# jbrea/BayesianOptimization.jl

Measured on AMD Instinct MI355X. Metric: acquisition-candidates/sec (N=3000,d=8), higher is better.
Workload: dtype f64

## Files before the change

### bayesianoptimization.jl_amd/csrc/kernels_score.hip

```cpp
#include "gemm_core.h"
#include "acq_log.h"

namespace bohip {

template <bool LOW>
__device__ __forceinline__ double cov_from_r_fast(int fam, double sigma2, double r) {
    if constexpr (LOW) {
        return matern_lo_k(fam, sigma2, r);
    } else {
        if (fam == FAM_M52) {
            const double R = sqrt(r), s = sqrt(5.0) * R;
            return sigma2 * (1.0 + s + 5.0 / 3.0 * r) * exp(-s);
        }
        return sigma2 * exp(-0.5 * r);
    }
}

struct KstarParts {
    const double* alpha;
    double* parts;
    int64_t ldp;
};
template <int DT, bool LOW>
__device__ __forceinline__ double kstar_value(const double (&xj)[DT], const double (&w)[DT], const double* xs, bool live, int fam,
                                              double sigma2) {
    double rr = 0.0;
#pragma unroll
    for (int k = 0; k < DT; ++k) {
        const double t = xj[k] - xs[k];
        rr += w[k] * (t * t);
    }
    return live ? cov_from_r_fast<LOW>(fam, sigma2, rr) : 0.0;
}
__device__ __forceinline__ void swap32(double a, double b, double& x, double& y) {
    const unsigned long long ua = (unsigned long long)__double_as_longlong(a), ub = (unsigned long long)__double_as_longlong(b);
    const auto lo = __builtin_amdgcn_permlane32_swap((unsigned)ua, (unsigned)ub, false, false);
    const auto hi = __builtin_amdgcn_permlane32_swap((unsigned)(ua >> 32), (unsigned)(ub >> 32), false, false);
    x = __longlong_as_double((long long)((unsigned long long)hi[0] << 32 | lo[0]));
    y = __longlong_as_double((long long)((unsigned long long)hi[1] << 32 | lo[1]));
}
template <int BIT>
__device__ __forceinline__ double halve_sum(double a, double b, int lane) {
    const bool up = lane & BIT;
    return (up ? b : a) + __shfl_xor(up ? a : b, BIT);
}
__device__ __forceinline__ void group_sum4(const double* p, int lane, double& sm, double& sa) {
    double x0, y0, x1, y1;
    swap32(p[0], p[2], x0, y0);
    swap32(p[1], p[3], x1, y1);
    sm = halve_sum<16>(x0 + y0, x1 + y1, lane);
    sa = halve_sum<16>(fabs(x0) + fabs(y0), fabs(x1) + fabs(y1), lane);
}
__device__ __forceinline__ double wave_finish(double s) {
    s += __shfl_xor(s, 2);
    s += __shfl_xor(s, 1);
    return s;
}

template <int DT, bool LOW, bool PARTS = false>
__global__ __launch_bounds__(256) void k_kstar(const double* __restrict__ X, int64_t N, int64_t Npad,
                                               const double* __restrict__ Xs, int64_t r_begin, int64_t r_end,
                                               KernelHyper hp, double* __restrict__ KsT, int64_t ldk, int rb, KstarParts kp) {
    __shared__ double xs_l[16 * DT];
    const int d = hp.d;
    const int64_t j = blockIdx.x * 256 + threadIdx.x;
    const int64_t r0 = r_begin + (int64_t)blockIdx.y * rb;
    const int64_t r1 = min(r0 + rb, r_end);
    for (int t = threadIdx.x; t < rb * DT; t += 256) {
        const int64_t r = r0 + t / DT;
        const int k = t % DT;
        xs_l[t] = (r < r1 && k < d) ? Xs[r * d + k] : 0.0;
    }
    double xj[DT], w[DT];
#pragma unroll
    for (int k = 0; k < DT; ++k) {
        xj[k] = (k < d && j < N) ? X[j * d + k] : 0.0;
        w[k] = k < d ? hp.il2[k] : 0.0;
    }
    __syncthreads();
    if (j >= Npad) return;
    const int nc = (int)(r1 - r0);
    if constexpr (PARTS) {
        const double aj = kp.alpha[j];
        const int lane = threadIdx.x & 63;
        double um[2], ua[2], tm0 = 0.0, ta0 = 0.0;
#pragma unroll
        for (int g = 0; g < 4; ++g) {
            double p[4];
#pragma unroll
            for (int i = 0; i < 4; ++i) {
                const int c = 4 * g + i;
                p[i] = 0.0;
                if (c < nc) {
                    const double v = kstar_value<DT, LOW>(xj, w, xs_l + c * DT, j < N, hp.fam, hp.sigma2);
                    KsT[(r0 + c - r_begin) * ldk + j] = v;
                    p[i] = aj * v;
                }
            }
            double tm, ta;
            group_sum4(p, lane, tm, ta);
            if (g & 1) {
                um[g >> 1] = halve_sum<8>(tm0, tm, lane);
                ua[g >> 1] = halve_sum<8>(ta0, ta, lane);
            } else {
                tm0 = tm;
                ta0 = ta;
            }
            __builtin_amdgcn_sched_barrier(0);
        }
        const double sm = wave_finish(halve_sum<4>(um[0], um[1], lane)), sa = wave_finish(halve_sum<4>(ua[0], ua[1], lane));
        const int c = 8 * ((lane >> 2) & 1) + 4 * ((lane >> 3) & 1) + 2 * (lane >> 5) + ((lane >> 4) & 1);
        if ((lane & 3) < 2 && c < nc) {
            const int64_t P = Npad >> 6;
            kp.parts[((int64_t)(lane & 1) * P + (j >> 6)) * kp.ldp + (r0 + c - r_begin)] = (lane & 1) ? sa : sm;
        }
    } else {
        for (int c = 0; c < nc; ++c) {
            const double v = kstar_value<DT, LOW>(xj, w, xs_l + c * DT, j < N, hp.fam, hp.sigma2);
            KsT[(r0 + c - r_begin) * ldk + j] = v;
        }
    }
}

template <int DT, bool LOW>
__global__ __launch_bounds__(256) void k_post_cov(const double* __restrict__ Xs, int64_t R, KernelHyper hp,
                                                  const double* __restrict__ VV, int64_t ldv,
                                                  double* __restrict__ cov, int64_t ldc) {
    const int d = hp.d;
    const int64_t s = blockIdx.x * 256 + threadIdx.x;
    if (s >= R) return;
    double xs[DT];
#pragma unroll
    for (int k = 0; k < DT; ++k) xs[k] = (k < d) ? Xs[s * d + k] : 0.0;
    const int64_t r0 = (int64_t)blockIdx.y * 16, r1 = min(R, r0 + 16);
    for (int64_t r = r0; r < r1; ++r) {
        double rr = 0.0;
#pragma unroll
        for (int k = 0; k < DT; ++k)
            if (k < d) {
                const double t = Xs[r * d + k] - xs[k];
                rr += hp.il2[k] * (t * t);
            }
        const double vv = (r >= s) ? VV[r * ldv + s] : VV[s * ldv + r];
        cov[r * ldc + s] = cov_from_r_fast<LOW>(hp.fam, hp.sigma2, rr) - vv;
    }
}

struct AcqParams {
    int acq;
    double p0, p1;
};
struct FuseParams {
    unsigned* tile_cnt;
    unsigned* total_cnt;
    Best* tile_best;
    int tiles_total;
    int T;
    int64_t R_total;
    double sigma2, beta;
    AcqParams ap;
    double *mu_out, *var_out, *score_out;
    Best* best_out;
    long long best_off;
    unsigned long long* clk;
    const unsigned* live;
};
__device__ void trigemm_fused_finish(const FuseParams& fz, int tile_g, int T, const double* q_part, int64_t ldq,
                                     const double* mu_raw);

#if BOHIP_TRACE
__device__ unsigned long long g_trace[6 * 8192];
#endif
constexpr int PIECE_WHOLE = 0, PIECE_UPPER_SOLO = 3;

__device__ __forceinline__ double sq_step(double s, double v) { return s + v * v; }
__device__ __forceinline__ double sq_tree(double s) {
    s += __shfl_xor(s, 8);
    s += __shfl_xor(s, 16);
    s += __shfl_xor(s, 32);
    return s;
}

__device__ __forceinline__ void trigemm_job(int rt, int mode, int ct, const double* __restrict__ W, int64_t ldw,
                                            const double* __restrict__ KsT, int64_t ldk, int NP, int64_t alpha_row,
                                            double* __restrict__ q_part, int64_t ldq, double* __restrict__ mu_raw, int64_t r_off,
                                            double* __restrict__ VT, int64_t ldv, const FuseParams& fz, double* smem, int tid) {
    constexpr int NJ = 4, CW = CTILE;
    double acc[8][NJ];
#pragma unroll
    for (int i = 0; i < 8; ++i)
#pragma unroll
        for (int j = 0; j < NJ; ++j) acc[i][j] = 0.0;
    const int64_t row_base = (int64_t)rt * TILE;
    const int active_rows = (int)min((int64_t)(mode == PIECE_WHOLE ? TILE : TILE / 2), alpha_row + 1 - row_base);
    const int tri_kc = rt * (TILE / KC);
    const int kc_end = mode == PIECE_WHOLE ? (rt + 1) * (TILE / KC) : tri_kc + 4;
    gemm_tile_loop_glds3_ks<NJ, BOHIP_ABL, true>(W + row_base * ldw, ldw, KsT + (int64_t)ct * CW * ldk, ldk, 0, kc_end, smem, acc,
                                                 active_rows, tri_kc, tid);
    const int lane = tid & 63, wave = tid >> 6, wr = (wave & 3) >> 1, wc = wave & 1;
    __syncthreads();
    double* red = smem;
    const bool rows_mine = mode == PIECE_WHOLE || wr == 0;
    if (wave < 4) {
#pragma unroll
    for (int nj = 0; nj < NJ; ++nj) {
        double s = 0.0;
#pragma unroll
        for (int mi = 0; mi < 8; ++mi) {
            const int64_t grow = row_base + acc_row(lane, wr, mi);
            const double v = acc[mi][nj];
            if (grow == alpha_row && rows_mine) {
                __hip_atomic_store(mu_raw + r_off + (int64_t)ct * CW + acc_col<NJ>(lane, wc, nj), v, __ATOMIC_RELAXED, __HIP_MEMORY_SCOPE_AGENT);
            } else {
                s = sq_step(s, v);
            }
            if (VT != nullptr && grow < alpha_row && rows_mine)
                VT[((int64_t)ct * CW + acc_col<NJ>(lane, wc, nj)) * ldv + grow] = v;
        }
        s = sq_tree(s);
        if (lane < 8) red[wr * CW + wc * 8 * NJ + 8 * nj + lane] = s;
    }
    }
    __syncthreads();
    if (tid < 2 * CW) {
        const int hh = tid >> 6, c = tid & (CW - 1);
        double* dst = q_part + (int64_t)(2 * rt + (mode == PIECE_WHOLE ? hh : 0)) * ldq + r_off + (int64_t)ct * CW + c;
        if (mode == PIECE_WHOLE || hh == 0) __hip_atomic_store(dst, red[hh * CW + c], __ATOMIC_RELAXED, __HIP_MEMORY_SCOPE_AGENT);
        else __hip_atomic_store(dst + ldq, 0.0, __ATOMIC_RELAXED, __HIP_MEMORY_SCOPE_AGENT);
    }
    if (fz.tile_cnt != nullptr) {
        __shared__ int s_last;
        const int tile_g = (int)(r_off / CW) + ct;
        asm volatile("s_waitcnt vmcnt(0)" ::: "memory");
        __syncthreads();
        if (tid == 0) s_last = atomicAdd(fz.tile_cnt + tile_g, 1u) == (unsigned)(NP - 1);
        __syncthreads();
        if (s_last && tid < 64) trigemm_fused_finish(fz, tile_g, fz.T, q_part, ldq, mu_raw);
    }
}

__global__ __launch_bounds__(GEMM_THREADS_8, 4) void k_trigemm_sq(const double* __restrict__ W, int64_t ldw,
                                                                  const double* __restrict__ KsT, int64_t ldk,
                                                                  const int* __restrict__ pieces, int NP, int CT, int64_t alpha_row,
                                                                  double* __restrict__ q_part, int64_t ldq,
                                                                  double* __restrict__ mu_raw, int64_t r_off,
                                                                  double* __restrict__ VT, int64_t ldv, FuseParams fz) {
    extern __shared__ __attribute__((aligned(16))) double smem[];
#if BOHIP_TRACE
    const unsigned long long t_start = wall_clock64(), c_start = clock64();
    struct TraceEnd {
        unsigned long long t0, c0;
        __device__ ~TraceEnd() {
            if (threadIdx.x == 0) {
                unsigned hw, xcc;
                asm volatile("s_getreg_b32 %0, hwreg(HW_REG_HW_ID)" : "=s"(hw));
                asm volatile("s_getreg_b32 %0, hwreg(HW_REG_XCC_ID)" : "=s"(xcc));
                unsigned long long* t = g_trace + 6 * (size_t)blockIdx.x;
                t[0] = t0; t[1] = wall_clock64(); t[2] = hw; t[3] = xcc; t[4] = c0; t[5] = clock64();
            }
        }
    } trace_end{t_start, c_start};
#endif
    const int xcd = blockIdx.x & 7, slot = blockIdx.x >> 3;
    const int n_local = (CT + 7) >> 3;
    const int ct = xcd + 8 * (slot % n_local);
    if (ct >= CT) return;
    if (fz.live != nullptr && ct * CTILE >= (int)*fz.live) return;
    const int piece = __builtin_amdgcn_readfirstlane(pieces[slot / n_local]);
    __shared__ unsigned long long s_clk[2];
    if (fz.clk != nullptr && blockIdx.x % 33 == 0 && threadIdx.x == 0) { s_clk[0] = clock64(); s_clk[1] = wall_clock64(); }
    trigemm_job(piece & 0xffff, piece >> 16, ct, W, ldw, KsT, ldk, NP, alpha_row, q_part, ldq, mu_raw, r_off, VT, ldv, fz, smem,
                    (int)threadIdx.x);
    if (fz.clk != nullptr && blockIdx.x % 33 == 0 && threadIdx.x == 0) {
        atomicAdd(fz.clk, (unsigned long long)clock64() - s_clk[0]);
        atomicAdd(fz.clk + 1, (unsigned long long)wall_clock64() - s_clk[1]);
    }
}

__device__ __forceinline__ void trigemm_job_rows64(int rt, int hh, int ct, const double* __restrict__ W, int64_t ldw,
                                                   const double* __restrict__ KsT, int64_t ldk, double* __restrict__ q_part,
                                                   int64_t ldq, double* smem, int tid) {
    constexpr int NJ = 4, CW = CTILE;
    double acc[8][NJ];
#pragma unroll
    for (int i = 0; i < 8; ++i)
#pragma unroll
        for (int j = 0; j < NJ; ++j) acc[i][j] = 0.0;
    const int64_t row_base = (int64_t)rt * TILE + 64 * hh;
    const int tri_kc = rt * (TILE / KC);
    const int kc_end = tri_kc + (hh == 0 ? 4 : 8);
    gemm_tile_loop_glds3_ks<NJ, BOHIP_ABL, true, true, true>(W + row_base * ldw, ldw, KsT + (int64_t)ct * CW * ldk, ldk, 0, kc_end, smem,
                                                             acc, TILE / 2, tri_kc, tid, hh);
    const int lane = tid & 63, wave = tid >> 6, wc = wave & 1;
    __syncthreads();
    double* red = smem;
    if (wave < 2) {
#pragma unroll
        for (int nj = 0; nj < NJ; ++nj) {
            double s = 0.0;
#pragma unroll
            for (int mi = 0; mi < 8; ++mi) s = sq_step(s, acc[mi][nj]);
            s = sq_tree(s);
            if (lane < 8) red[wc * 8 * NJ + 8 * nj + lane] = s;
        }
    }
    __syncthreads();
    if (tid < CW)
        __hip_atomic_store(q_part + (int64_t)(2 * rt + hh) * ldq + (int64_t)ct * CW + tid, red[tid], __ATOMIC_RELAXED, __HIP_MEMORY_SCOPE_AGENT);
}

__global__ __launch_bounds__(GEMM_THREADS_8, 4) void k_trigemm_sq_pa(const double* __restrict__ W, int64_t ldw,
                                                                     const double* __restrict__ KsT, int64_t ldk,
                                                                     const int* __restrict__ jobs, int CT, double* __restrict__ q_part,
                                                                     int64_t ldq, unsigned long long* clk) {
    extern __shared__ __attribute__((aligned(16))) double smem[];
#if BOHIP_TRACE
    const unsigned long long t_start = wall_clock64(), c_start = clock64();
    struct TraceEnd {
        unsigned long long t0, c0;
        __device__ ~TraceEnd() {
            if (threadIdx.x == 0) {
                unsigned hw, xcc;
                asm volatile("s_getreg_b32 %0, hwreg(HW_REG_HW_ID)" : "=s"(hw));
                asm volatile("s_getreg_b32 %0, hwreg(HW_REG_XCC_ID)" : "=s"(xcc));
                unsigned long long* t = g_trace + 6 * (size_t)blockIdx.x;
                t[0] = t0; t[1] = wall_clock64(); t[2] = hw; t[3] = xcc; t[4] = c0; t[5] = clock64();
            }
        }
    } trace_end{t_start, c_start};
#endif
    const int xcd = blockIdx.x & 7, slot = blockIdx.x >> 3;
    const int n_local = (CT + 7) >> 3;
    const int ct = xcd + 8 * (slot % n_local);
    if (ct >= CT) return;
    const int job = __builtin_amdgcn_readfirstlane(jobs[slot / n_local]);
    __shared__ unsigned long long s_clk[2];
    if (clk != nullptr && blockIdx.x % 33 == 0 && threadIdx.x == 0) { s_clk[0] = clock64(); s_clk[1] = wall_clock64(); }
    trigemm_job_rows64(job & 0xffff, job >> 16, ct, W, ldw, KsT, ldk, q_part, ldq, smem, (int)threadIdx.x);
    if (clk != nullptr && blockIdx.x % 33 == 0 && threadIdx.x == 0) {
        atomicAdd(clk, (unsigned long long)clock64() - s_clk[0]);
        atomicAdd(clk + 1, (unsigned long long)wall_clock64() - s_clk[1]);
    }
}

__global__ __launch_bounds__(256) void k_split_combine_v(const double* __restrict__ PT, int64_t plane, int64_t ldp, int kz,
                                                         int64_t N, double* __restrict__ q, double* __restrict__ mu_raw,
                                                         double* __restrict__ VT, int64_t ldv) {
    __shared__ double red[256];
    const int r = blockIdx.x;
    const double* base = PT + (int64_t)r * ldp;
    double s = 0.0;
    for (int64_t i = threadIdx.x; i <= N; i += 256) {
        const int nsl = (int)(((i >> 7) + 1) * (TILE / KC) + kz - 1) / kz;
        double v = 0.0;
        for (int sl = 0; sl < nsl; ++sl) v += base[(int64_t)sl * plane + i];
        if (i < N) {
            s += v * v;
            if (VT) VT[(int64_t)r * ldv + i] = v;
        } else {
            mu_raw[r] = v;
        }
    }
    red[threadIdx.x] = s;
    __syncthreads();
    for (int o = 128; o > 0; o >>= 1) {
        if (threadIdx.x < o) red[threadIdx.x] += red[threadIdx.x + o];
        __syncthreads();
    }
    if (threadIdx.x == 0) q[r] = red[0];
}
__global__ __launch_bounds__(256) void k_split_combine_u(const double* __restrict__ PU, int64_t plane, int64_t ldp, int kz,
                                                         int nslices, int64_t N, double* __restrict__ UT, int64_t ldu) {
    const int r = blockIdx.x;
    const double* base = PU + (int64_t)r * ldp;
    for (int64_t j = threadIdx.x; j < N; j += 256) {
        const int s0 = (int)((j >> 7) * (TILE / KC)) / kz;
        double v = 0.0;
        for (int sl = s0; sl < nslices; ++sl) v += base[(int64_t)sl * plane + j];
        UT[(int64_t)r * ldu + j] = v;
    }
}

template <bool LOGEI = true>
__device__ __forceinline__ double acq_eval(const AcqParams& a, double mu, double s2) {
#pragma clang fp contract(off)
    switch (a.acq) {
        case ACQ_EI: {
            const double tau = a.p0;
            if (s2 == 0.0) return mu > tau ? mu - tau : 0.0;
            const double D = mu - tau;
            const double cdf = 1.0 / 2.0 * (1.0 + erf(D / sqrt(2.0 * s2)));
            const double pdf = 1.0 / sqrt(2.0 * M_PI * s2) * exp(-(D * D) / (2.0 * s2));
            return D * cdf + sqrt(s2) * pdf;
        }
        case ACQ_PI: {
            const double tau = a.p0;
            if (s2 == 0.0) return mu > tau ? 1.0 : 0.0;
            return 1.0 / 2.0 * (1.0 + erf((mu - tau) / sqrt(2.0 * s2)));
        }
        case ACQ_UCB:
            return mu + a.p0 * sqrt(s2);
        case ACQ_MI:
            return mu + a.p0 * (sqrt(s2 + a.p1) - sqrt(a.p1));
        case ACQ_LOGEI:
            if constexpr (LOGEI) return logei_value(mu, s2, a.p0);
            else return NAN;
        default:
            return mu;
    }
}

__device__ __forceinline__ bool better(double v, long long i, double bv, long long bi) {
    if (i < 0) return false;
    if (bi < 0) return v > -INFINITY;
    return v > bv || (v == bv && i < bi);
}
__device__ __forceinline__ void block_argmax(double& v, long long& i, Best* sh) {
    for (int o = 32; o > 0; o >>= 1) {
        const double ov = __shfl_xor(v, o);
        const long long oi = __shfl_xor(i, o);
        if (better(ov, oi, v, i)) { v = ov; i = oi; }
    }
    const int lane = threadIdx.x & 63, wave = threadIdx.x >> 6;
    if (lane == 0) { sh[wave].val = v; sh[wave].idx = i; }
    __syncthreads();
    if (threadIdx.x == 0) {
        for (int w = 1; w < (int)(blockDim.x >> 6); ++w)
            if (better(sh[w].val, sh[w].idx, v, i)) { v = sh[w].val; i = sh[w].idx; }
    }
}

__device__ void trigemm_fused_finish(const FuseParams& fz, int tile_g, int T, const double* q_part, int64_t ldq,
                                     const double* mu_raw) {
#pragma clang fp contract(off)
    const int lane = threadIdx.x & 63;
    const int64_t r = (int64_t)tile_g * CTILE + lane;
    double v = -INFINITY;
    long long idx = -1;
    if (r < fz.R_total) {
        double q = 0.0;
        for (int t = 0; t < T; ++t)
            q += __hip_atomic_load(q_part + (int64_t)(2 * t) * ldq + r, __ATOMIC_RELAXED, __HIP_MEMORY_SCOPE_AGENT) +
                 __hip_atomic_load(q_part + (int64_t)(2 * t + 1) * ldq + r, __ATOMIC_RELAXED, __HIP_MEMORY_SCOPE_AGENT);
        double s2 = fz.sigma2 - q;
        if (s2 < 0.0) s2 = 0.0;
        const double mu = fz.beta + __hip_atomic_load(mu_raw + r, __ATOMIC_RELAXED, __HIP_MEMORY_SCOPE_AGENT);
        if (fz.mu_out) fz.mu_out[r] = mu;
        if (fz.var_out) fz.var_out[r] = s2;
        const double f = acq_eval(fz.ap, mu, s2);
        if (fz.score_out) fz.score_out[r] = f;
        if (f > -INFINITY) { v = f; idx = r; }
    }
    for (int o = 32; o > 0; o >>= 1) {
        const double ov = __shfl_xor(v, o);
        const long long oi = __shfl_xor(idx, o);
        if (better(ov, oi, v, idx)) { v = ov; idx = oi; }
    }
    int last = 0;
    if (lane == 0) {
        fz.tile_cnt[tile_g] = 0u;
        if (fz.best_out) {
            __hip_atomic_store(&fz.tile_best[tile_g].val, idx >= 0 ? v : -INFINITY, __ATOMIC_RELAXED, __HIP_MEMORY_SCOPE_AGENT);
            __hip_atomic_store(&fz.tile_best[tile_g].idx, idx, __ATOMIC_RELAXED, __HIP_MEMORY_SCOPE_AGENT);
            asm volatile("s_waitcnt vmcnt(0)" ::: "memory");
            last = atomicAdd(fz.total_cnt, 1u) == (unsigned)(fz.tiles_total - 1);
        }
    }
    last = __shfl(last, 0);
    if (!last) return;
    v = -INFINITY;
    idx = -1;
    for (int i = lane; i < fz.tiles_total; i += 64) {
        const double bv = __hip_atomic_load(&fz.tile_best[i].val, __ATOMIC_RELAXED, __HIP_MEMORY_SCOPE_AGENT);
        const long long bi = __hip_atomic_load(&fz.tile_best[i].idx, __ATOMIC_RELAXED, __HIP_MEMORY_SCOPE_AGENT);
        if (better(bv, bi, v, idx)) { v = bv; idx = bi; }
    }
    for (int o = 32; o > 0; o >>= 1) {
        const double ov = __shfl_xor(v, o);
        const long long oi = __shfl_xor(idx, o);
        if (better(ov, oi, v, idx)) { v = ov; idx = oi; }
    }
    if (lane == 0) {
        *fz.total_cnt = 0u;
        fz.best_out->val = idx >= 0 ? v : -INFINITY;
        fz.best_out->idx = idx >= 0 ? idx + fz.best_off : -1;
    }
}

__global__ __launch_bounds__(256) void k_score(const double* __restrict__ q_part, int64_t ldq, int T,
                                               const double* __restrict__ mu_raw, int64_t R, double sigma2,
                                               double beta, AcqParams ap, double* __restrict__ mu_out,
                                               double* __restrict__ var_out, double* __restrict__ score_out,
                                               Best* __restrict__ block_best) {
#pragma clang fp contract(off)
    __shared__ Best sh[4];
    const int64_t r = blockIdx.x * 256 + threadIdx.x;
    double v = -INFINITY;
    long long idx = -1;
    if (r < R) {
        double q = 0.0;
        for (int t = 0; t < T; ++t) q += q_part[(int64_t)(2 * t) * ldq + r] + q_part[(int64_t)(2 * t + 1) * ldq + r];
        if (T == 0) q = q_part[r];
        double s2 = sigma2 - q;
        if (s2 < 0.0) s2 = 0.0;
        const double mu = beta + mu_raw[r];
        if (mu_out) mu_out[r] = mu;
        if (var_out) var_out[r] = s2;
        const double f = acq_eval(ap, mu, s2);
        if (score_out) score_out[r] = f;
        if (f > -INFINITY) { v = f; idx = r; }
    }
    if (block_best) {
        block_argmax(v, idx, sh);
        if (threadIdx.x == 0) { block_best[blockIdx.x].val = idx >= 0 ? v : -INFINITY; block_best[blockIdx.x].idx = idx; }
    }
}

__global__ __launch_bounds__(256) void k_argmax_final(const Best* __restrict__ in, int n, Best* __restrict__ out, long long idx_off) {
    __shared__ Best sh[4];
    double v = -INFINITY;
    long long idx = -1;
    for (int i = threadIdx.x; i < n; i += 256)
        if (better(in[i].val, in[i].idx, v, idx)) { v = in[i].val; idx = in[i].idx; }
    block_argmax(v, idx, sh);
    if (threadIdx.x == 0) { out->val = idx >= 0 ? v : -INFINITY; out->idx = idx >= 0 ? idx + idx_off : -1; }
}

struct PruneBound {
    const double* parts;
    int64_t P, ldp, Npad;
    const double* q;
    int64_t ldq, R;
    int m;
    double sigma2, beta;
    AcqParams ap;
    double* ub;
};
__global__ __launch_bounds__(64) void k_prune_bound(PruneBound pb) {
#pragma clang fp contract(off)
    const int64_t r = (int64_t)blockIdx.x * 64 + threadIdx.x;
    if (r >= pb.R) return;
    double mu = 0.0, sa = 0.0;
    for (int64_t w0 = 0; w0 < pb.P; w0 += 16) {
        double a[16], b[16];
#pragma unroll
        for (int i = 0; i < 16; ++i) {
            const int64_t w = min(w0 + i, pb.P - 1);
            a[i] = pb.parts[w * pb.ldp + r];
            b[i] = pb.parts[(pb.P + w) * pb.ldp + r];
        }
#pragma unroll
        for (int i = 0; i < 16; ++i)
            if (w0 + i < pb.P) { mu += a[i]; sa += b[i]; }
    }
    double qp = 0.0;
    for (int t = 0; t < pb.m; ++t) qp += pb.q[(int64_t)(2 * t) * pb.ldq + r] + pb.q[(int64_t)(2 * t + 1) * pb.ldq + r];
    double s2 = pb.sigma2 - qp;
    if (s2 < 0.0) s2 = 0.0;
    const double n = (double)(pb.Npad + 64), un = n * 0x1p-53, gam = un / (1.0 - un);
    double y = mu + (4.0 * gam * sa + 0x1p-1000);
    y += fabs(y) * 0x1p-52 + 0x1p-1000;
    const double mu_up = pb.beta + y;
    const AcqParams& ap = pb.ap;
    double ub;
    switch (ap.acq) {
        case ACQ_EI: {
            const double D = mu_up - ap.p0;
            const double f = acq_eval(ap, mu_up, D <= 0.0 ? fmin(s2, 1.0) : 1.0);
            ub = f + 0x1p-38 * (1.0 + sqrt(pb.sigma2) + fmax(D, 0.0) + fabs(f));
            break;
        }
        case ACQ_PI:
            ub = (mu_up - ap.p0 >= 0.0 ? 1.0 : acq_eval(ap, mu_up, s2)) + 0x1p-38;
            break;
        case ACQ_UCB:
        case ACQ_MI: {
            const double sb = ap.p0 >= 0.0 ? s2 : 0.0;
            const double f = acq_eval(ap, mu_up, sb);
            const double roots = ap.acq == ACQ_UCB ? sqrt(sb) : sqrt(sb + fabs(ap.p1)) + sqrt(fabs(ap.p1));
            ub = f + 0x1p-38 * (fabs(mu_up) + fabs(ap.p0) * roots + 0x1p-1000);
            break;
        }
        case ACQ_LOGEI: {
            const double f = acq_eval(ap, mu_up, s2);
            ub = f == -INFINITY ? f : f + 0x1p-38 * (1.0 + fabs(f));
            break;
        }
        default:
            ub = mu_up;
    }
    pb.ub[r] = ub;
}

__device__ __forceinline__ double prune_key(double v) { return v != v ? INFINITY : v; }
__device__ __forceinline__ unsigned long long prune_key_bits(double v) {
    const double k = prune_key(v);
    const unsigned long long b = k == 0.0 ? 0ull : (unsigned long long)__double_as_longlong(k);
    return (b >> 63) ? ~b : b | 0x8000000000000000ull;
}
constexpr int SELECT_THREADS = 1024, SELECT_PER = 8;
constexpr int PRUNE_ARRIVE = 4;
__global__ __launch_bounds__(SELECT_THREADS) void k_prune_select(const double* __restrict__ ub, int64_t R, int k1, int* __restrict__ list1,
                                                                 int* __restrict__ mark, unsigned* __restrict__ cnt, Best* __restrict__ rec) {
    __shared__ uint4 hist[3][64];
    __shared__ unsigned long long red[2 * SELECT_THREADS / 64];
    __shared__ unsigned tot[SELECT_THREADS / 64];
    const int t = threadIdx.x, lane = t & 63, wave = t >> 6;
    const int per = (int)((R + SELECT_THREADS - 1) / SELECT_THREADS);
    unsigned long long key[SELECT_PER];
    unsigned long long kmax = 0ull, kmin = ~0ull;
#pragma unroll
    for (int i = 0; i < SELECT_PER; ++i) {
        const int64_t r = (int64_t)t * per + i;
        key[i] = (i < per && r < R) ? prune_key_bits(ub[r]) : 0ull;
        if (key[i]) { kmax = max(kmax, key[i]); kmin = min(kmin, key[i]); }
    }
    for (int o = 32; o > 0; o >>= 1) {
        kmax = max(kmax, __shfl_xor(kmax, o));
        kmin = min(kmin, __shfl_xor(kmin, o));
    }
    if (lane == 0) { red[2 * wave] = kmax; red[2 * wave + 1] = kmin; }
    if (t < 128) (&hist[0][0])[t] = make_uint4(0u, 0u, 0u, 0u);
    __syncthreads();
    for (int w = 0; w < SELECT_THREADS / 64; ++w) { kmax = max(kmax, red[2 * w]); kmin = min(kmin, red[2 * w + 1]); }
    unsigned long long prefix = kmax;
    int hb = kmax == kmin ? 0 : 64 - __clzll((long long)(kmax ^ kmin)), k = k1;
    for (int pass = 0; hb > 0; ++pass) {
        const int wd = hb < 8 ? hb : 8, shift = hb - wd;
        unsigned* h = reinterpret_cast<unsigned*>(hist[pass % 3]);
#pragma unroll
        for (int i = 0; i < SELECT_PER; ++i)
            if (key[i] && (hb == 64 || (key[i] >> hb) == (prefix >> hb))) atomicAdd(h + ((unsigned)(key[i] >> shift) & ((1u << wd) - 1u)), 1u);
        __syncthreads();
        if (t < 64) hist[(pass + 2) % 3][t] = make_uint4(0u, 0u, 0u, 0u);
        const uint4 c4 = hist[pass % 3][63 - lane];
        const unsigned c[4] = {c4.w, c4.z, c4.y, c4.x};
        unsigned incl = c[0] + c[1] + c[2] + c[3];
        for (int o = 1; o < 64; o <<= 1) {
            const unsigned u = __shfl_up(incl, o);
            if (lane >= o) incl += u;
        }
        unsigned run = incl - (c[0] + c[1] + c[2] + c[3]);
        int found = -1, knew = 0, all = 0;
#pragma unroll
        for (int i = 0; i < 4; ++i) {
            if (run < (unsigned)k && (unsigned)k <= run + c[i]) { found = 255 - 4 * lane - i; knew = k - (int)run; all = knew == (int)c[i]; }
            run += c[i];
        }
        const unsigned long long who = __ballot(found >= 0);
        const int src = __ffsll((long long)who) - 1;
        const int digit = __shfl(found, src);
        k = __shfl(knew, src);
        all = __shfl(all, src);
        const unsigned long long low = hb == 64 ? ~0ull : (1ull << hb) - 1ull;
        prefix = (prefix & ~low) | (unsigned long long)digit << shift;
        hb = shift;
        if (all) break;
    }
    const unsigned long long thr = prefix >> hb;
    int ngt = 0, neq = 0;
#pragma unroll
    for (int i = 0; i < SELECT_PER; ++i) { ngt += key[i] && (key[i] >> hb) > thr; neq += key[i] && (key[i] >> hb) == thr; }
    const unsigned mine = (unsigned)ngt | (unsigned)neq << 16;
    unsigned incl = mine;
    for (int o = 1; o < 64; o <<= 1) {
        const unsigned u = __shfl_up(incl, o);
        if (lane >= o) incl += u;
    }
    if (lane == 63) tot[wave] = incl;
    __syncthreads();
    for (int w = 0; w < wave; ++w) incl += tot[w];
    int g = (int)((incl - mine) & 0xffffu), e = (int)((incl - mine) >> 16);
#pragma unroll
    for (int i = 0; i < SELECT_PER; ++i) {
        if (!key[i]) continue;
        const int64_t r = (int64_t)t * per + i;
        const bool gt = (key[i] >> hb) > thr, eq = (key[i] >> hb) == thr, in = gt || (eq && e < k);
        if (in) list1[g + min(e, k)] = (int)r;
        mark[r] = in;
        g += gt;
        e += eq;
    }
    if (t == 0) {
        cnt[0] = (unsigned)k1;
        cnt[1] = 0u;
        cnt[PRUNE_ARRIVE] = 0u;
        cnt[PRUNE_ARRIVE + 1] = 0u;
        rec->val = -INFINITY;
        rec->idx = -1;
    }
}

__global__ __launch_bounds__(256) void k_prune_gather(const int* __restrict__ list, const unsigned* __restrict__ cnt,
                                                      const double* __restrict__ src, int64_t ld, int64_t ncols, double* __restrict__ dst,
                                                      int sq_min, unsigned* __restrict__ live_out) {
    const int i = blockIdx.x, n = (int)*cnt;
    if (i == 0 && threadIdx.x == 0) *live_out = n > sq_min ? (unsigned)n : 0u;
    if (i >= n || n <= sq_min) return;
    const d2* s = reinterpret_cast<const d2*>(src + (int64_t)list[i] * ld);
    d2* d = reinterpret_cast<d2*>(dst + (int64_t)i * ld);
    for (int64_t j = threadIdx.x; j < ncols / 2; j += 256) d[j] = s[j];
}

struct PruneFinish {
    const int* list;
    const unsigned* cnt;
    const double *q, *q2, *mu2;
    int64_t ldq, ldq2;
    int m, T;
    double sigma2, beta;
    AcqParams ap;
    Best* rec;
    Best* best_out;
    long long best_off;
    unsigned* stat;
    const double* ub;
    const int* mark;
    int64_t R;
    int* list2;
    unsigned* cnt2;
};
template <int NT>
__device__ __forceinline__ void prune_finish_body(const PruneFinish& pf, Best* sh, double* tail_L, unsigned* tail_n) {
#pragma clang fp contract(off)
    const int n = (int)*pf.cnt;
    double v = -INFINITY;
    long long idx = -1;
    for (int i = threadIdx.x; i < n; i += NT) {
        const int64_t r = pf.list[i];
        double q = 0.0;
        for (int t0 = 0; t0 < pf.T; t0 += 8) {
            double a[8], b[8];
#pragma unroll
            for (int u = 0; u < 8; ++u) {
                const int t = min(t0 + u, pf.T - 1);
                const double* src = t < pf.m ? pf.q + r : pf.q2 + i;
                const int64_t ld = t < pf.m ? pf.ldq : pf.ldq2;
                a[u] = src[(int64_t)(2 * t) * ld];
                b[u] = src[(int64_t)(2 * t + 1) * ld];
            }
#pragma unroll
            for (int u = 0; u < 8; ++u)
                if (t0 + u < pf.T) q += a[u] + b[u];
        }
        double s2 = pf.sigma2 - q;
        if (s2 < 0.0) s2 = 0.0;
        const double mu = pf.beta + pf.mu2[i];
        const double f = acq_eval(pf.ap, mu, s2);
        if (better(f, r, v, idx)) { v = f; idx = r; }
    }
    block_argmax(v, idx, sh);
    const bool last_round = !pf.list2;
    if (threadIdx.x == 0) {
        const Best b = *pf.rec;
        if (better(b.val, b.idx, v, idx)) { v = b.val; idx = b.idx; }
        pf.rec->val = idx >= 0 ? v : -INFINITY;
        pf.rec->idx = idx;
        if (pf.best_out && last_round) {
            pf.best_out->val = idx >= 0 ? v : -INFINITY;
            pf.best_out->idx = idx >= 0 ? idx + pf.best_off : -1;
        }
        if (pf.stat && last_round) *pf.stat = (unsigned)n;
        *tail_L = idx >= 0 ? v : -INFINITY;
        *tail_n = 0u;
    }
    if (last_round) return;
    __syncthreads();
    const double L = *tail_L;
    for (int64_t r0 = threadIdx.x; r0 < pf.R; r0 += 8 * NT) {
        int mk[8];
        double u[8];
#pragma unroll
        for (int i = 0; i < 8; ++i) {
            const int64_t r = min(r0 + NT * i, pf.R - 1);
            mk[i] = pf.mark[r];
            u[i] = pf.ub[r];
        }
#pragma unroll
        for (int i = 0; i < 8; ++i)
            if (r0 + NT * i < pf.R && !mk[i] && !(u[i] < L)) pf.list2[atomicAdd(tail_n, 1u)] = (int)(r0 + NT * i);
    }
    __syncthreads();
    if (threadIdx.x == 0) {
        const unsigned n2 = *tail_n;
        *pf.cnt2 = n2;
        if (n2 == 0u) {
            if (pf.best_out) {
                pf.best_out->val = idx >= 0 ? v : -INFINITY;
                pf.best_out->idx = idx >= 0 ? idx + pf.best_off : -1;
            }
            if (pf.stat) *pf.stat = 0u;
        }
    }
}
__global__ __launch_bounds__(256) void k_prune_finish(PruneFinish pf) {
    __shared__ Best sh[4];
    __shared__ double tail_L;
    __shared__ unsigned tail_n;
    prune_finish_body<256>(pf, sh, &tail_L, &tail_n);
}

constexpr int RS_COLS = 8, RS_WAVES = 8, RS_THREADS = 64 * RS_WAVES, RS_DEPTH = 8;
constexpr int RS_RG = 16 / RS_WAVES;
constexpr int RS_BUF = (64 + RS_COLS) * KC;
constexpr int RS_LDS_BYTES = RS_DEPTH * RS_BUF * 8;
struct RowsParams {
    const double* W;
    int64_t ldw;
    const double* KsT;
    int64_t ldk;
    const int* list;
    const unsigned* cnt;
    int cnt_max;
    const int* halves;
    int NH, G;
    int64_t alpha_row;
    double* q;
    int64_t ldq;
    double* mu;
    int finish;
    unsigned* arrive;
    PruneFinish pf;
};
__global__ __launch_bounds__(RS_THREADS) void k_trigemm_rows(RowsParams rp) {
    __shared__ double xch[2 * 64 * RS_COLS];
    __shared__ double vb[64 * RS_COLS];
    const int xcd = blockIdx.x & 7, slot = blockIdx.x >> 3;
    const int hi = xcd + 8 * (slot / rp.G), grp0 = slot % rp.G;
    const int n = (int)*rp.cnt;
    if (hi >= rp.NH || n > rp.cnt_max || grp0 * RS_COLS >= n) return;
    const int code = __builtin_amdgcn_readfirstlane(rp.halves[hi]);
    const int rt = code & 0xffff, hh = (code >> 16) & 1;
    const bool solo = (code >> 17) & 1;
    const int tid = threadIdx.x, lane = tid & 63, wave = __builtin_amdgcn_readfirstlane(tid >> 6);
    const int h = wave / (RS_WAVES / 2), wq = wave % (RS_WAVES / 2);
    const int k = lane >> 4, b = (lane >> 2) & 3;
    const int tri_kc = 8 * rt, kc_end = tri_kc + (hh == 0 ? 4 : 8);
    const int g0 = 8 * hh + RS_RG * wq;
    extern __shared__ __attribute__((aligned(16))) double rs_ring[];
    const int prow = lane >> 3, sseg = (lane & 7) ^ prow;
    const bool has_b = wave == 0;
    const double* a_src0 = rp.W + ((int64_t)rt * TILE + 64 * hh + 8 * wave + prow) * rp.ldw + 2 * sseg;
    const double* b_src = nullptr;
    auto issue = [&](int kc, int buf) {
        kc = min(kc, kc_end - 1);
        double* d = rs_ring + buf * RS_BUF;
        __builtin_amdgcn_global_load_lds((gbl_void_ptr)(a_src0 + (int64_t)kc * KC), (lds_void_ptr)(d + 8 * wave * KC), 16, 0, 0);
        if (has_b)
            __builtin_amdgcn_global_load_lds((gbl_void_ptr)(b_src + (int64_t)kc * KC), (lds_void_ptr)(d + 64 * KC), 16, 0, 0);
    };
    auto wait_left = [&](auto left) {
        constexpr int L = decltype(left)::value;
        if (has_b) asm volatile("s_waitcnt vmcnt(%0)" ::"n"(2 * L) : "memory");
        else asm volatile("s_waitcnt vmcnt(%0)" ::"n"(L) : "memory");
    };
    const int rr = 4 * (b >> 1) + (lane & 3), cc = 4 * (b & 1) + (lane & 3), S = 4 * h + k;
    const uint32_t ring0 = (uint32_t)(uintptr_t)(__attribute__((address_space(3))) const double*)rs_ring;
    const uint32_t fa = ring0 + (uint32_t)(((8 * RS_RG * wq + rr) * KC + 2 * (S ^ rr)) * 8);
    const uint32_t fb = ring0 + (uint32_t)(((64 + cc) * KC + 2 * (S ^ cc)) * 8);
    auto frags = [&](int buf, d2 (&av)[RS_RG], d2 (&bv)[1]) {
        const uint32_t off = (uint32_t)(buf * RS_BUF * 8);
        av[0] = ds_read128<0>(fa + off);
        av[1] = ds_read128<1024>(fa + off);
        bv[0] = ds_read128<0>(fb + off);
    };
    auto landed = [&](d2 (&av)[RS_RG], d2 (&bv)[1]) {
        asm volatile("s_waitcnt lgkmcnt(0)" : "+v"(av[0]), "+v"(av[1]), "+v"(bv[0]));
    };
    double acc[RS_RG][1], acc2[RS_RG][1];
    auto run = [&](auto solo_tag) {
        constexpr bool SOLO = decltype(solo_tag)::value;
#pragma unroll
        for (int i = 0; i < RS_RG; ++i)
#pragma unroll
            for (int j = 0; j < 1; ++j) acc[i][j] = acc2[i][j] = 0.0;
        auto mmas = [&](int kc, const d2 (&av)[RS_RG], const d2 (&bv)[1]) {
            const int skip = kc >= tri_kc ? 2 * (kc - tri_kc) + h - g0 : 0;
#pragma unroll
            for (int i = 0; i < RS_RG; ++i) {
                if (skip > i) continue;
                if constexpr (SOLO) {
                    mma_row<1, 1>(av[i], bv, acc[i]);
                    mma_row<1, 2>(av[i], bv, acc2[i]);
                } else {
                    mma_row<1, 0>(av[i], bv, acc[i]);
                }
            }
        };
        static_assert(RS_DEPTH % 2 == 0, "a pair of chunks per barrier: the ring turns in pairs");
#pragma unroll
        for (int p = 0; p < RS_DEPTH - 1; ++p) issue(p, p);
        d2 av0[RS_RG], bv0[1], av1[RS_RG], bv1[1];
        wait_left(std::integral_constant<int, RS_DEPTH - 2>{});
        __builtin_amdgcn_s_barrier();
        __builtin_amdgcn_sched_barrier(0);
        frags(0, av0, bv0);
        landed(av0, bv0);
        __builtin_amdgcn_sched_barrier(0);
        int cur = 0;
        for (int kc = 0; kc < kc_end; kc += 2) {
            wait_left(std::integral_constant<int, RS_DEPTH - 4>{});
            __builtin_amdgcn_s_barrier();
            __builtin_amdgcn_sched_barrier(0);
            const int prev = cur == 0 ? RS_DEPTH - 1 : cur - 1, b1 = cur + 1, b2 = cur + 2 == RS_DEPTH ? 0 : cur + 2;
            issue(kc + RS_DEPTH - 1, prev);
            issue(kc + RS_DEPTH, cur);
            frags(b1, av1, bv1);
            __builtin_amdgcn_sched_barrier(0);
            mmas(kc, av0, bv0);
            landed(av1, bv1);
            __builtin_amdgcn_sched_barrier(0);
            frags(b2, av0, bv0);
            __builtin_amdgcn_sched_barrier(0);
            mmas(kc + 1, av1, bv1);
            landed(av0, bv0);
            __builtin_amdgcn_sched_barrier(0);
            cur = b2;
        }
        asm volatile("s_waitcnt vmcnt(0)" ::: "memory");
    };
    for (int grp = grp0; grp * RS_COLS < n; grp += rp.G) {
    const int ib = grp * RS_COLS + prow;
    b_src = rp.KsT + (int64_t)(ib < n ? rp.list[ib] : rp.list[0]) * rp.ldk + 2 * sseg;
    if (solo) run(std::true_type{});
    else run(std::false_type{});
    if (h == 1) {
#pragma unroll
        for (int i = 0; i < RS_RG; ++i)
#pragma unroll
            for (int j = 0; j < 1; ++j) {
                xch[((wq * RS_RG + i)  + j) * 64 + lane] = acc[i][j];
                xch[64 * RS_COLS + ((wq * RS_RG + i)  + j) * 64 + lane] = acc2[i][j];
            }
    }
    __syncthreads();
    if (h == 0) {
#pragma unroll
        for (int i = 0; i < RS_RG; ++i)
#pragma unroll
            for (int j = 0; j < 1; ++j) {
                const double a1 = xch[((wq * RS_RG + i)  + j) * 64 + lane];
                double v = acc[i][j] + a1;
                if (solo) {
                    const double o1 = xch[64 * RS_COLS + ((wq * RS_RG + i)  + j) * 64 + lane];
                    v = v + (acc2[i][j] + o1);
                }
                const int row = 8 * (RS_RG * wq + i) + 4 * (b >> 1) + k, col = 8 * j + 4 * (b & 1) + (lane & 3);
                vb[row * RS_COLS + col] = v;
            }
    }
    __syncthreads();
    if (wave == 0) {
    const int col = 8 * wave + 4 * (b & 1) + (lane & 3), i_list = grp * RS_COLS + col;
    const int64_t row_base = (int64_t)rt * TILE + 64 * hh;
    double s = 0.0;
#pragma unroll
    for (int mi = 0; mi < 8; ++mi) {
        const int row = 8 * mi + 4 * (b >> 1) + k;
        const double v = vb[row * RS_COLS + col];
        if (row_base + row == rp.alpha_row) {
            if (i_list < n) rp.mu[i_list] = v;
        } else {
            s = sq_step(s, v);
        }
    }
    s = sq_tree(s);
    if (lane < 8 && i_list < n) {
        rp.q[(int64_t)(2 * rt + hh) * rp.ldq + i_list] = s;
        if (solo) rp.q[(int64_t)(2 * rt + 1) * rp.ldq + i_list] = 0.0;
    }
    asm volatile("s_waitcnt vmcnt(0)" ::: "memory");
    }
    __syncthreads();
    }
    if (!rp.finish) return;
    unsigned* flag = reinterpret_cast<unsigned*>(xch + 64);
    if (tid == 0) {
        __builtin_amdgcn_fence(__ATOMIC_RELEASE, "agent");
        asm volatile("s_waitcnt vmcnt(0)" ::: "memory");
        const unsigned want = (unsigned)rp.NH * (unsigned)min(rp.G, (n + RS_COLS - 1) / RS_COLS);
        const bool last = __hip_atomic_fetch_add(rp.arrive, 1u, __ATOMIC_RELAXED, __HIP_MEMORY_SCOPE_AGENT) == want - 1u;
        if (last) __hip_atomic_store(rp.arrive, 0u, __ATOMIC_RELAXED, __HIP_MEMORY_SCOPE_AGENT);
        *flag = last;
    }
    __syncthreads();
    if (!*flag) return;
    if (tid == 0) {
        __builtin_amdgcn_fence(__ATOMIC_ACQUIRE, "agent");
        asm volatile("s_waitcnt vmcnt(0)" ::: "memory");
    }
    __syncthreads();
    prune_finish_body<RS_THREADS>(rp.pf, reinterpret_cast<Best*>(xch), xch + 32, reinterpret_cast<unsigned*>(xch + 40));
}

__global__ __launch_bounds__(256) void k_reduce_records(const Best* __restrict__ all, int nrec, int S, Best* __restrict__ out) {
    const int s = blockIdx.x * 256 + threadIdx.x;
    if (s >= S) return;
    double v = -INFINITY;
    long long idx = -1;
    for (int r = 0; r < nrec; ++r) {
        const Best b = all[(int64_t)r * S + s];
        if (better(b.val, b.idx, v, idx)) { v = b.val; idx = b.idx; }
    }
    out[s].val = idx >= 0 ? v : -INFINITY;
    out[s].idx = idx;
}

template <bool LOGEI = true>
__device__ __forceinline__ void acq_partials(const AcqParams& a, double mu, double s2, double& dmu, double& ds2) {
    const double inv_sqrt_2pi = 0.3989422804014327;
    switch (a.acq) {
        case ACQ_EI: {
            if (s2 == 0.0) { dmu = mu > a.p0 ? 1.0 : 0.0; ds2 = 0.0; return; }
            const double D = mu - a.p0, s = sqrt(s2), z = D / s;
            const double Phi = 0.5 * (1.0 + erf(z / sqrt(2.0))), phi = inv_sqrt_2pi * exp(-0.5 * z * z);
            dmu = Phi + D * phi / s - z * phi / s;
            ds2 = (D * phi - z * phi) * (-z / (2.0 * s2));
            return;
        }
        case ACQ_PI: {
            if (s2 == 0.0) { dmu = 0.0; ds2 = 0.0; return; }
            const double D = mu - a.p0, s = sqrt(s2), z = D / s, phi = inv_sqrt_2pi * exp(-0.5 * z * z);
            dmu = phi / s;
            ds2 = phi * (-z / (2.0 * s2));
            return;
        }
        case ACQ_UCB: dmu = 1.0; ds2 = s2 > 0.0 ? a.p0 / (2.0 * sqrt(s2)) : 0.0; return;
        case ACQ_MI: dmu = 1.0; ds2 = a.p0 / (2.0 * sqrt(s2 + a.p1)); return;
        case ACQ_LOGEI:
            if constexpr (LOGEI) { const LogEIPartials g = logei_partials(mu, s2, a.p0); dmu = g.dmu; ds2 = g.ds2; }
            else { dmu = NAN; ds2 = NAN; }
            return;
        default: dmu = 1.0; ds2 = 0.0; return;
    }
}

__global__ __launch_bounds__(256) void k_acq_eval(AcqParams ap, int64_t n, const double* __restrict__ mu, const double* __restrict__ var,
                                                  double* __restrict__ value, double* __restrict__ dmu, double* __restrict__ dvar) {
    const int64_t i = (int64_t)blockIdx.x * 256 + threadIdx.x;
    if (i >= n) return;
    value[i] = acq_eval(ap, mu[i], var[i]);
    if (dmu) acq_partials(ap, mu[i], var[i], dmu[i], dvar[i]);
}

__device__ __forceinline__ void posterior_like_small_finish(double sigma2, double beta, double q, double mu_raw, double& mu, double& s2) {
#pragma clang fp contract(off)
    s2 = sigma2 - q;
    if (s2 < 0.0) s2 = 0.0;
    mu = beta + mu_raw;
}
constexpr int grad_finish_waves(int DT, bool LOW) { return DT <= 2 ? 8 : DT <= 4 ? 7 - LOW : DT <= 8 ? 5 - LOW : DT <= 16 ? 3 : DT <= 32 ? 2 : 1; }
template <int DT, bool LOW>
__global__ __launch_bounds__(256, grad_finish_waves(DT, LOW)) void k_grad_finish(const double* __restrict__ X, int64_t N,
                                                     const double* __restrict__ Xs, int64_t r_begin, int64_t r_end,
                                                     KernelHyper hp, const double* __restrict__ alpha,
                                                     const double* __restrict__ UT, int64_t ldu,
                                                     const double* __restrict__ mu, const double* __restrict__ var,
                                                     AcqParams ap, double* __restrict__ grad,
                                                     double* __restrict__ parts, unsigned* __restrict__ counters) {
    __shared__ double red[4][2 * DT];
    __shared__ int is_last;
    constexpr int PS = 2 * DT;
    const int lane = threadIdx.x & 63, wave = threadIdx.x >> 6;
    const int64_t r = r_begin + blockIdx.x;
    if (r >= r_end) return;
    const int d = hp.d, S = gridDim.y, sp = blockIdx.y;
    const int64_t len = ((N + S - 1) / S + 255) / 256 * 256;
    const int64_t j_lo = sp * len, j_hi = min(N, j_lo + len);
    const double* xs = Xs + r * d;
    double gm[DT], gv[DT];
#pragma unroll
    for (int k = 0; k < DT; ++k) { gm[k] = 0.0; gv[k] = 0.0; }
    const double* u = UT + (r - r_begin) * ldu;
    for (int64_t j = j_lo + threadIdx.x; j < j_hi; j += 256) {
        double t[DT], rr = 0.0;
#pragma unroll
        for (int k = 0; k < DT; ++k)
            if (k < d) {
                t[k] = xs[k] - X[j * d + k];
                rr += hp.il2[k] * (t[k] * t[k]);
            }
        double fac;
        if constexpr (LOW) {
            fac = matern_lo_fx(hp.fam, hp.sigma2, rr);
        } else if (hp.fam == FAM_M52) {
            const double s = sqrt(5.0) * sqrt(rr);
            fac = -(5.0 / 3.0) * hp.sigma2 * (1.0 + s) * exp(-s);
        } else {
            fac = -(hp.sigma2 * exp(-0.5 * rr));
        }
        const double a = alpha[j], uj = u[j];
#pragma unroll
        for (int k = 0; k < DT; ++k)
            if (k < d) {
                const double dk = fac * t[k] * hp.il2[k];
                gm[k] += dk * a;
                gv[k] += dk * uj;
            }
    }
#pragma unroll
    for (int k = 0; k < DT; ++k)
        if (k < d) {
            double a = gm[k], b = gv[k];
            for (int o = 32; o > 0; o >>= 1) { a += __shfl_xor(a, o); b += __shfl_xor(b, o); }
            if (lane == 0) { red[wave][2 * k] = a; red[wave][2 * k + 1] = b; }
        }
    __syncthreads();
    if (S > 1) {
        double* mine = parts + ((int64_t)blockIdx.x * S + sp) * PS;
        if (threadIdx.x < 2 * d)
            __hip_atomic_store(mine + threadIdx.x, (red[0][threadIdx.x] + red[1][threadIdx.x]) + (red[2][threadIdx.x] + red[3][threadIdx.x]),
                               __ATOMIC_RELAXED, __HIP_MEMORY_SCOPE_AGENT);
        asm volatile("s_waitcnt vmcnt(0)" ::: "memory");
        __syncthreads();
        if (threadIdx.x == 0) is_last = atomicAdd(&counters[blockIdx.x], 1u) == (unsigned)(S - 1);
        __syncthreads();
        if (!is_last) return;
        if (threadIdx.x == 0) counters[blockIdx.x] = 0u;
    }
    if (threadIdx.x < d) {
        const int k = threadIdx.x;
        double a, b;
        if (S > 1) {
            a = 0.0; b = 0.0;
            const double* all = parts + (int64_t)blockIdx.x * S * PS;
            for (int q = 0; q < S; ++q) {
                a += __hip_atomic_load(all + q * PS + 2 * k, __ATOMIC_RELAXED, __HIP_MEMORY_SCOPE_AGENT);
                b += __hip_atomic_load(all + q * PS + 2 * k + 1, __ATOMIC_RELAXED, __HIP_MEMORY_SCOPE_AGENT);
            }
        } else {
            a = (red[0][2 * k] + red[1][2 * k]) + (red[2][2 * k] + red[3][2 * k]);
            b = (red[0][2 * k + 1] + red[1][2 * k + 1]) + (red[2][2 * k + 1] + red[3][2 * k + 1]);
        }
        double dmu, ds2;
        const double m = mu[r], v = var[r];
        acq_partials(ap, m, v, dmu, ds2);
        grad[r * d + k] = dmu * a + (v > 0.0 ? ds2 * (-2.0 * b) : 0.0);
    }
}

constexpr int GC = 2;
template <int DT, bool LOW>
__global__ __launch_bounds__(256) void k_grad_finish_tiled(const double* __restrict__ X, int64_t N,
                                                           const double* __restrict__ Xs, int64_t r_begin, int64_t r_end,
                                                           KernelHyper hp, const double* __restrict__ alpha,
                                                           const double* __restrict__ UT, int64_t ldu,
                                                           const double* __restrict__ mu, const double* __restrict__ var,
                                                           AcqParams ap, double* __restrict__ grad) {
    __shared__ double red[4][GC][2 * DT];
    const int lane = threadIdx.x & 63, wave = threadIdx.x >> 6;
    const int64_t rb = r_begin + (int64_t)blockIdx.x * GC;
    if (rb >= r_end) return;
    const int d = hp.d, nc = (int)min((int64_t)GC, r_end - rb);
    double xs[GC][DT], gm[GC][DT], gv[GC][DT], w[DT];
#pragma unroll
    for (int k = 0; k < DT; ++k) w[k] = k < d ? hp.il2[k] : 0.0;
#pragma unroll
    for (int c = 0; c < GC; ++c)
#pragma unroll
        for (int k = 0; k < DT; ++k) {
            xs[c][k] = (c < nc && k < d) ? Xs[(rb + c) * d + k] : 0.0;
            gm[c][k] = 0.0;
            gv[c][k] = 0.0;
        }
    for (int64_t j = threadIdx.x; j < N; j += 256) {
        double xj[DT];
#pragma unroll
        for (int k = 0; k < DT; ++k) xj[k] = k < d ? X[j * d + k] : 0.0;
        const double a = alpha[j];
#pragma unroll
        for (int c = 0; c < GC; ++c) {
            double t[DT], rr = 0.0;
#pragma unroll
            for (int k = 0; k < DT; ++k) {
                t[k] = xs[c][k] - xj[k];
                rr += w[k] * (t[k] * t[k]);
            }
            double fac;
            if constexpr (LOW) {
                fac = matern_lo_fx(hp.fam, hp.sigma2, rr);
            } else if (hp.fam == FAM_M52) {
                const double s = sqrt(5.0) * sqrt(rr);
                fac = -(5.0 / 3.0) * hp.sigma2 * (1.0 + s) * exp(-s);
            } else {
                fac = -(hp.sigma2 * exp(-0.5 * rr));
            }
            const double uj = c < nc ? UT[(rb + c - r_begin) * ldu + j] : 0.0;
#pragma unroll
            for (int k = 0; k < DT; ++k) {
                const double dk = fac * t[k] * w[k];
                gm[c][k] += dk * a;
                gv[c][k] += dk * uj;
            }
        }
    }
#pragma unroll
    for (int c = 0; c < GC; ++c)
#pragma unroll
        for (int k = 0; k < DT; ++k)
            if (k < d) {
                double a = gm[c][k], b = gv[c][k];
                for (int o = 32; o > 0; o >>= 1) { a += __shfl_xor(a, o); b += __shfl_xor(b, o); }
                if (lane == 0) { red[wave][c][2 * k] = a; red[wave][c][2 * k + 1] = b; }
            }
    __syncthreads();
    if ((int)threadIdx.x < GC * d) {
        const int c = threadIdx.x / d, k = threadIdx.x % d;
        if (c < nc) {
            const int64_t r = rb + c;
            const double a = (red[0][c][2 * k] + red[1][c][2 * k]) + (red[2][c][2 * k] + red[3][c][2 * k]);
            const double b = (red[0][c][2 * k + 1] + red[1][c][2 * k + 1]) + (red[2][c][2 * k + 1] + red[3][c][2 * k + 1]);
            double dmu, ds2;
            const double m = mu[r], v = var[r];
            acq_partials(ap, m, v, dmu, ds2);
            grad[r * d + k] = dmu * a + (v > 0.0 ? ds2 * (-2.0 * b) : 0.0);
        }
    }
}

__host__ __device__ inline uint64_t splitmix64(uint64_t x) {
    x += 0x9E3779B97F4A7C15ull;
    x = (x ^ (x >> 30)) * 0xBF58476D1CE4E5B9ull;
    x = (x ^ (x >> 27)) * 0x94D049BB133111EBull;
    return x ^ (x >> 31);
}
__host__ __device__ inline double thompson_normal(uint64_t seed, int64_t s, int64_t j) {
    const uint64_t h = splitmix64(seed ^ splitmix64((uint64_t)s * 0xD1B54A32D192ED03ull + (uint64_t)j));
    const uint64_t h2 = splitmix64(h);
    const double u1 = ((double)(h >> 11) + 1.0) * (1.0 / 9007199254740993.0);
    const double u2 = (double)(h2 >> 11) * (1.0 / 9007199254740992.0);
    return sqrt(-2.0 * log(u1)) * cos(2.0 * M_PI * u2);
}

__global__ __launch_bounds__(256) void k_thompson(const double* __restrict__ mu, const double* __restrict__ var,
                                                  int64_t R, uint64_t seed, int64_t j0, Best* __restrict__ out,
                                                  long long idx_off) {
#pragma clang fp contract(off)
    __shared__ Best sh[4];
    const int64_t s = blockIdx.x;
    double v = -INFINITY;
    long long idx = -1;
    for (int64_t r = threadIdx.x; r < R; r += 256) {
        const double f = mu[r] + sqrt(var[r]) * thompson_normal(seed, s, j0 + r);
        if (better(f, r, v, idx)) { v = f; idx = r; }
    }
    block_argmax(v, idx, sh);
    if (threadIdx.x == 0) { out[s].val = idx >= 0 ? v : -INFINITY; out[s].idx = idx >= 0 ? idx + idx_off : -1; }
}

}
```

Before: 29.60 million.

## Replace agent fences with relaxed atomics and prefetch loads in prune finish

Drops the release and acquire agent-scope fences around the last-block election and makes the cross-block stores and loads of q, q2 and mu relaxed agent-scope atomics instead. It also splits the q/q2 accumulation into two separate software-prefetched loops and hoists the first tail-pass mark/ub loads ahead of the scoring loop. The aim is to cut fence and cache-flush latency and hide load latency in the single-block finish. Relaxed atomics without fences give weaker ordering guarantees, so this risks reading stale data from other blocks.

Measured after the change: 30.02 million (median of 4 runs). Within noise of the previous version (+1.4%).

```diff
diff --git a/bayesianoptimization.jl_amd/csrc/kernels_score.hip b/bayesianoptimization.jl_amd/csrc/kernels_score.hip
--- a/bayesianoptimization.jl_amd/csrc/kernels_score.hip
+++ b/bayesianoptimization.jl_amd/csrc/kernels_score.hip
@@ -720,37 +720,71 @@
     int* list2;
     unsigned* cnt2;
 };
+constexpr int FINISH_A = 8, FINISH_B = 8;
 template <int NT>
 __device__ __forceinline__ void prune_finish_body(const PruneFinish& pf, Best* sh, double* tail_L, unsigned* tail_n) {
 #pragma clang fp contract(off)
     const int n = (int)*pf.cnt;
+    const bool last_round = !pf.list2;
+    int mk[8];
+    double u8[8];
+    auto tail_load = [&](int64_t r0) {
+#pragma unroll
+        for (int i = 0; i < 8; ++i) {
+            const int64_t r = min(r0 + NT * i, pf.R - 1);
+            mk[i] = pf.mark[r];
+            u8[i] = pf.ub[r];
+        }
+    };
+    if (!last_round && (int64_t)threadIdx.x < pf.R) tail_load(threadIdx.x);
     double v = -INFINITY;
     long long idx = -1;
     for (int i = threadIdx.x; i < n; i += NT) {
         const int64_t r = pf.list[i];
+        const double mu_raw = __hip_atomic_load(pf.mu2 + i, __ATOMIC_RELAXED, __HIP_MEMORY_SCOPE_AGENT);
         double q = 0.0;
-        for (int t0 = 0; t0 < pf.T; t0 += 8) {
-            double a[8], b[8];
-#pragma unroll
-            for (int u = 0; u < 8; ++u) {
+        double aa[FINISH_A], ab[FINISH_A], ba[FINISH_B], bb[FINISH_B];
+        auto load_a = [&](int t0) {
+#pragma unroll
+            for (int u = 0; u < FINISH_A; ++u) {
+                const int t = min(t0 + u, pf.m - 1);
+                aa[u] = pf.q[(int64_t)(2 * t) * pf.ldq + r];
+                ab[u] = pf.q[(int64_t)(2 * t + 1) * pf.ldq + r];
+            }
+        };
+        auto load_b = [&](int t0) {
+#pragma unroll
+            for (int u = 0; u < FINISH_B; ++u) {
                 const int t = min(t0 + u, pf.T - 1);
-                const double* src = t < pf.m ? pf.q + r : pf.q2 + i;
-                const int64_t ld = t < pf.m ? pf.ldq : pf.ldq2;
-                a[u] = src[(int64_t)(2 * t) * ld];
-                b[u] = src[(int64_t)(2 * t + 1) * ld];
-            }
-#pragma unroll
-            for (int u = 0; u < 8; ++u)
-                if (t0 + u < pf.T) q += a[u] + b[u];
+                ba[u] = __hip_atomic_load(pf.q2 + (int64_t)(2 * t) * pf.ldq2 + i, __ATOMIC_RELAXED, __HIP_MEMORY_SCOPE_AGENT);
+                bb[u] = __hip_atomic_load(pf.q2 + (int64_t)(2 * t + 1) * pf.ldq2 + i, __ATOMIC_RELAXED, __HIP_MEMORY_SCOPE_AGENT);
+            }
+        };
+        load_a(0);
+        load_b(pf.m);
+        for (int t0 = 0;;) {
+#pragma unroll
+            for (int u = 0; u < FINISH_A; ++u)
+                if (t0 + u < pf.m) q += aa[u] + ab[u];
+            t0 += FINISH_A;
+            if (t0 >= pf.m) break;
+            load_a(t0);
+        }
+        for (int t0 = pf.m;;) {
+#pragma unroll
+            for (int u = 0; u < FINISH_B; ++u)
+                if (t0 + u < pf.T) q += ba[u] + bb[u];
+            t0 += FINISH_B;
+            if (t0 >= pf.T) break;
+            load_b(t0);
         }
         double s2 = pf.sigma2 - q;
         if (s2 < 0.0) s2 = 0.0;
-        const double mu = pf.beta + pf.mu2[i];
+        const double mu = pf.beta + mu_raw;
         const double f = acq_eval(pf.ap, mu, s2);
         if (better(f, r, v, idx)) { v = f; idx = r; }
     }
     block_argmax(v, idx, sh);
-    const bool last_round = !pf.list2;
     if (threadIdx.x == 0) {
         const Best b = *pf.rec;
         if (better(b.val, b.idx, v, idx)) { v = b.val; idx = b.idx; }
@@ -768,17 +802,10 @@
     __syncthreads();
     const double L = *tail_L;
     for (int64_t r0 = threadIdx.x; r0 < pf.R; r0 += 8 * NT) {
-        int mk[8];
-        double u[8];
-#pragma unroll
-        for (int i = 0; i < 8; ++i) {
-            const int64_t r = min(r0 + NT * i, pf.R - 1);
-            mk[i] = pf.mark[r];
-            u[i] = pf.ub[r];
-        }
+        if (r0 != (int64_t)threadIdx.x) tail_load(r0);
 #pragma unroll
         for (int i = 0; i < 8; ++i)
-            if (r0 + NT * i < pf.R && !mk[i] && !(u[i] < L)) pf.list2[atomicAdd(tail_n, 1u)] = (int)(r0 + NT * i);
+            if (r0 + NT * i < pf.R && !mk[i] && !(u8[i] < L)) pf.list2[atomicAdd(tail_n, 1u)] = (int)(r0 + NT * i);
     }
     __syncthreads();
     if (threadIdx.x == 0) {
@@ -959,15 +986,16 @@
         const int row = 8 * mi + 4 * (b >> 1) + k;
         const double v = vb[row * RS_COLS + col];
         if (row_base + row == rp.alpha_row) {
-            if (i_list < n) rp.mu[i_list] = v;
+            if (i_list < n) __hip_atomic_store(rp.mu + i_list, v, __ATOMIC_RELAXED, __HIP_MEMORY_SCOPE_AGENT);
         } else {
             s = sq_step(s, v);
         }
     }
     s = sq_tree(s);
     if (lane < 8 && i_list < n) {
-        rp.q[(int64_t)(2 * rt + hh) * rp.ldq + i_list] = s;
-        if (solo) rp.q[(int64_t)(2 * rt + 1) * rp.ldq + i_list] = 0.0;
+        __hip_atomic_store(rp.q + (int64_t)(2 * rt + hh) * rp.ldq + i_list, s, __ATOMIC_RELAXED, __HIP_MEMORY_SCOPE_AGENT);
+        if (solo)
+            __hip_atomic_store(rp.q + (int64_t)(2 * rt + 1) * rp.ldq + i_list, 0.0, __ATOMIC_RELAXED, __HIP_MEMORY_SCOPE_AGENT);
     }
     asm volatile("s_waitcnt vmcnt(0)" ::: "memory");
     }
@@ -976,8 +1004,6 @@
     if (!rp.finish) return;
     unsigned* flag = reinterpret_cast<unsigned*>(xch + 64);
     if (tid == 0) {
-        __builtin_amdgcn_fence(__ATOMIC_RELEASE, "agent");
-        asm volatile("s_waitcnt vmcnt(0)" ::: "memory");
         const unsigned want = (unsigned)rp.NH * (unsigned)min(rp.G, (n + RS_COLS - 1) / RS_COLS);
         const bool last = __hip_atomic_fetch_add(rp.arrive, 1u, __ATOMIC_RELAXED, __HIP_MEMORY_SCOPE_AGENT) == want - 1u;
         if (last) __hip_atomic_store(rp.arrive, 0u, __ATOMIC_RELAXED, __HIP_MEMORY_SCOPE_AGENT);
@@ -985,11 +1011,6 @@
     }
     __syncthreads();
     if (!*flag) return;
-    if (tid == 0) {
-        __builtin_amdgcn_fence(__ATOMIC_ACQUIRE, "agent");
-        asm volatile("s_waitcnt vmcnt(0)" ::: "memory");
-    }
-    __syncthreads();
     prune_finish_body<RS_THREADS>(rp.pf, reinterpret_cast<Best*>(xch), xch + 32, reinterpret_cast<unsigned*>(xch + 40));
 }
 
```
